# bayesian-object-tracking/dbot_ros

Measured on AMD Instinct MI355X. Metric: particle-likelihoods/sec @640x480, higher is better.
Workload: dtype f64; 1 GPU; C1: 2000 particles/GPU x loglikes(update=true), 640x480 synthetic depth frame, mesh m1 (5120 triangles), parents=permutation, 30-frame moving-object sequence, likelihood precision f64, window planes, inputs resident in HBM; particles_per_gpu=2000, triangles=5120

## Files before the change

dbot_ros_amd/csrc/rbsensor_kernels.hip:

```cpp
#pragma once
#include <hip/hip_runtime.h>
#include <math.h>
#include <stdint.h>

#include "rbs_device.h"
#include "rbs_math.h"

namespace rbs {

#ifndef RBS_TILE_PX
#define RBS_TILE_PX 11008
#endif
#ifndef RBS_COPY_UNROLL
#define RBS_COPY_UNROLL 8
#endif
#ifndef RBS_BIG_THRESH
#define RBS_BIG_THRESH 96
#endif

#ifndef RBS_BLOCK
#define RBS_BLOCK 256
#endif
constexpr int kBlock = RBS_BLOCK;
constexpr int kTilePx = RBS_TILE_PX;
// ... 1046 lines not shown
    RBS_EVAL_BATCH(qn);
#undef RBS_EVAL_BATCH
    RBS_TICK(3);
    if (draw && threadIdx.x == 0) ticket = atomicAdd(&P.ctr_this[1], 1);
    const double total = block_reduce_sum(ll, m.red);
    RBS_TICK(4);
    return total;
}

__device__ inline bool raster_writes(const DevParams& P, int particle, const int4& q, int row, int col)
{
    if (!(row >= q.y && row < q.w && col >= q.x && col < q.z)) return false;
    if (P.groups == nullptr) return true;
    const Groups* G = P.groups + particle;
    const int ng = G->n;
    for (int g = 0; g < ng; ++g) {
        const int4 r = G->rect[g];
        if (row >= r.y && row < r.w && col >= r.x && col < r.z) return true;
    }
    return false;
}

template <int VEC>
__device__ inline void copy_band(const DevParams& P, int particle, int band, Rect r)
{
    const int row0 = band * P.band_rows;
    const int row1 = min(P.rows, row0 + P.band_rows);
    if (row0 >= row1) return;
    const int parent = P.parents[particle];
    if ((unsigned)parent >= (unsigned)P.slots) return;
    const float* __restrict__ src = parent_plane(P, parent) + (size_t)row0 * P.cols;
    float* __restrict__ dst = P.occ_dst + (size_t)particle * P.plane_stride + (size_t)row0 * P.cols;
    const float alpha = P.alpha, beta = P.beta, bg_new = P.bg_new;

    if (VEC == 4) {
        const int W4 = P.cols >> 2;
        const int n4 = (row1 - row0) * W4;
        const floatx4* __restrict__ s4 = reinterpret_cast<const floatx4*>(src);
        floatx4* __restrict__ d4 = reinterpret_cast<floatx4*>(dst);
        const int qstep = kBlock / W4, rstep = kBlock - qstep * W4;
        int row = row0 + (int)threadIdx.x / W4;
        int c4 = (int)threadIdx.x - ((int)threadIdx.x / W4) * W4;
        for (int base = threadIdx.x; base < n4; base += kBlock * kCopyUnroll) {
            floatx4 v[kCopyUnroll];
            bool ok[kCopyUnroll];
#pragma unroll
            for (int k = 0; k < kCopyUnroll; ++k) {
                const int idx = base + k * kBlock;
                const int col = c4 << 2;
                ok[k] = idx < n4 && !raster_writes(P, particle, make_int4(r.x0, r.y0, r.x1, r.y1), row, col);
                if (ok[k]) v[k] = __builtin_nontemporal_load(&s4[idx]);
                c4 += rstep; row += qstep;
                if (c4 >= W4) { c4 -= W4; ++row; }
            }
#pragma unroll
            for (int k = 0; k < kCopyUnroll; ++k) {
                if (!ok[k]) continue;
                floatx4 w;
                w.x = occ_step(alpha, beta, v[k].x, bg_new);
                w.y = occ_step(alpha, beta, v[k].y, bg_new);
                w.z = occ_step(alpha, beta, v[k].z, bg_new);
                w.w = occ_step(alpha, beta, v[k].w, bg_new);
                __builtin_nontemporal_store(w, &d4[base + k * kBlock]);
            }
        }
    } else {
        const int W = P.cols;
        const int n1 = (row1 - row0) * W;
        for (int idx = threadIdx.x; idx < n1; idx += kBlock) {
            const int lr = idx / W;
            const int row = row0 + lr, col = idx - lr * W;
            if (raster_writes(P, particle, make_int4(r.x0, r.y0, r.x1, r.y1), row, col)) continue;
            dst[idx] = occ_step(alpha, beta, src[idx], bg_new);
        }
    }
}

constexpr int kPrepPerBlock = 8;

__device__ inline void compose_pose(const double* __restrict__ d, const double* __restrict__ d0, double* __restrict__ out)
{
    double Rd[9], R0[9];
    rbd::rotvec_to_matrix(d + 3, Rd);
    rbd::rotvec_to_matrix(d0 + 3, R0);
    rbd::matmul3(Rd, R0, out);
#pragma unroll
    for (int k = 0; k < 3; ++k) out[9 + k] = d[k] + d0[k];
}

template <bool DELTAS = false>
__device__ inline void prep_particles(const DevParams& P, int block, int* __restrict__ rects, int update)
{
    __shared__ int cnts[kPrepPerBlock + 1];
    const int w = threadIdx.x >> 6, lane = threadIdx.x & 63;
    const int i = block * kPrepPerBlock + w;
    const bool live = i < P.n;
    const int parent_early = live ? P.indices[i] : -1;
    Rect r = {0, 0, 0, 0};
    int cnt = 0;
    __shared__ int4 gr_s[kPrepPerBlock][kMaxBodies];
    __shared__ unsigned gm_s[kPrepPerBlock][kMaxBodies];
    __shared__ Groups G_s[kPrepPerBlock];
    __shared__ int ys_s[kPrepPerBlock][2 * kMaxGroups + 4];
    int4* const gr = gr_s[w];
    unsigned* const gm = gm_s[w];
    Groups& G = G_s[w];
    if (lane == 0) G.n = 0;
    const int cap_px = min(P.tile_w * P.tile_h, P.tile_px);
    if (DELTAS && live) {
        const int B = P.n_bodies;
        double* dstp = const_cast<double*>(P.poses) + (size_t)i * 12 * B;
        for (int b = lane; b < B; b += 64) {
            double d[6], d0[6], out[12];
#pragma unroll
            for (int k = 0; k < 6; ++k) { d[k] = P.deltas_src[((size_t)i * B + b) * 6 + k]; d0[k] = P.deltas_src[((size_t)P.n * B + b) * 6 + k]; }
            compose_pose(d, d0, out);
#pragma unroll
            for (int k = 0; k < 12; ++k) dstp[12 * b + k] = out[k];
        }
        __threadfence_block();
    } else if (P.poses_src && live) {
        const int m = 12 * P.n_bodies;
        double* dstp = const_cast<double*>(P.poses) + (size_t)i * m;
        const double* srcp = P.poses_src + (size_t)i * m;
        for (int k = lane; k < m; k += 64) dstp[k] = srcp[k];
        __threadfence_block();
    }
    if (live && P.groups == nullptr) {
        r = particle_rect(P, P.poses + (size_t)i * 12 * P.n_bodies);
        const TileGrid tg = tile_grid(r.x1 - r.x0, r.y1 - r.y0, P.tile_w, cap_px);
        cnt = r.x1 > r.x0 ? tg.nx * tg.ny : 1;
    } else if (live) {
        int ng = 0;
        for (int b = 0; b < P.n_bodies; ++b) {
            const Rect br = bodies_rect(P, P.poses + (size_t)i * 12 * P.n_bodies, b, b + 1);
            if (br.x1 > br.x0) {
                if (lane == 0) { gr[ng] = make_int4(br.x0, br.y0, br.x1, br.y1); gm[ng] = 1u << b; }
                ++ng;
            }
        }
        __builtin_amdgcn_wave_barrier();
        for (bool changed = true; changed;) {
            changed = false;
            for (int a = 0; a < ng && !changed; ++a)
                for (int c = a + 1; c < ng && !changed; ++c) {
                    const int4 A = gr[a], C = gr[c];
                    if (A.x < C.z && C.x < A.z && A.y < C.w && C.y < A.w) {
                        const int4 last = gr[ng - 1];
                        const unsigned ma = gm[a], mc = gm[c], ml = gm[ng - 1];
                        __builtin_amdgcn_wave_barrier();
                        if (lane == 0) {
                            gr[a] = make_int4(min(A.x, C.x), min(A.y, C.y), max(A.z, C.z), max(A.w, C.w));
                            gm[a] = ma | mc;
                            if (c != ng - 1) { gr[c] = last; gm[c] = ml; }
                        }
                        __builtin_amdgcn_wave_barrier();
                        --ng;
                        changed = true;
                    }
                }
        }
        if (ng > kMaxGroups) {
            int4 U = gr[0];
            unsigned mu = gm[0];
            for (int c = 1; c < ng; ++c) {
                const int4 C = gr[c];
                U = make_int4(min(U.x, C.x), min(U.y, C.y), max(U.z, C.z), max(U.w, C.w));
                mu |= gm[c];
            }
            __builtin_amdgcn_wave_barrier();
            if (lane == 0) { gr[0] = U; gm[0] = mu; }
            __builtin_amdgcn_wave_barrier();
            ng = 1;
        }
        if (lane == 0) G.n = ng;
        if (ng > 0) { const int4 g0 = gr[0]; r = Rect{g0.x, g0.y, g0.z, g0.w}; }
        for (int g = 0; g < ng; ++g) {
            const int4 R = gr[g];
            const TileGrid tg = tile_grid(R.z - R.x, R.w - R.y, P.tile_w, cap_px);
            if (lane == 0) { G.rect[g] = R; G.mask[g] = gm[g]; G.first[g] = cnt; }
            cnt += tg.nx * tg.ny;
            r.x0 = min(r.x0, R.x); r.y0 = min(r.y0, R.y);
            r.x1 = max(r.x1, R.z); r.y1 = max(r.y1, R.w);
        }
        if (ng == 0) cnt = 1;
    }
    if (lane == 0) cnts[w] = cnt;
    __syncthreads();
    if (threadIdx.x == 0) {
        int total = 0;
        for (int k = 0; k < kPrepPerBlock; ++k) { const int c = cnts[k]; cnts[k] = total; total += c; }
        cnts[kPrepPerBlock] = total ? atomicAdd(&P.ctr_this[0], total) : 0;
    }
    __syncthreads();
    if (!live || lane != 0) return;
    reinterpret_cast<int4*>(rects)[i] = make_int4(r.x0, r.y0, r.x1, r.y1);
    if (P.groups) {
        Groups* out = P.groups + i;
        out->n = G.n;
        for (int g = 0; g < G.n; ++g) { out->rect[g] = G.rect[g]; out->first[g] = G.first[g]; out->mask[g] = G.mask[g]; }
    }
    P.done[i] = 0;
    const int parent = parent_early;
    P.parents[i] = parent;
    const int first = cnts[kPrepPerBlock] + cnts[w];
    P.item_range[i] = make_int2(first, cnt);
    for (int k = 0; k < cnt; ++k) P.item_particle[first + k] = i;
    if (update && P.windowed) {
        const int4 rw = r.x1 > r.x0 ? make_int4(r.x0, r.y0, r.x1, r.y1) : make_int4(P.cols, P.rows, 0, 0);
        int4 pw = make_int4(P.cols, P.rows, 0, 0);
        if ((unsigned)parent < (unsigned)P.slots) pw = parent_window(P, parent);
        int4 u = make_int4(min(pw.x, rw.x), min(pw.y, rw.y), max(pw.z, rw.z), max(pw.w, rw.w));
        if (P.rebase_box) {
            const int4 bw = *P.rebase_box;
            u = make_int4(min(u.x, bw.x), min(u.y, bw.y), max(u.z, bw.z), max(u.w, bw.w));
        }
        int4 seed = rw;
        if (P.slab_px) {
            const long area = u.z > u.x && u.w > u.y ? (long)(u.z - u.x) * (long)(u.w - u.y) : 0;
            if (area > (long)P.err[1]) atomicMax(P.err + 1, (int)min(area, 0x7fffffffL));
            if (area > (long)P.slab_px) {
                P.parents[i] = -1;
                u = make_int4(P.cols, P.rows, 0, 0);
                seed = u;
                atomicExch(P.err, 1);
            }
            P.reg_dst[i] = u;
        }
        P.win_used[i] = u;
        P.win_dst[i] = seed;
        if (P.strips && P.groups) {
            Strips* S = P.strips + i;
            int* ys = ys_s[w];
            int ny = 0, ns = 0, total = 0;
            const int ng_ = G.n;
            if (u.z > u.x && u.w > u.y) {
                ys[ny++] = u.y;
                for (int g = 0; g < ng_; ++g) {
                    const int4 R = G.rect[g];
                    for (int e = 0; e < 2; ++e) {
                        const int y = min(max(e ? R.w : R.y, u.y), u.w);
                        int k = ny;
                        while (k > 0 && ys[k - 1] > y) --k;
                        if (k > 0 && ys[k - 1] == y) continue;
                        for (int m = ny; m > k; --m) ys[m] = ys[m - 1];
                        ys[k] = y; ++ny;
                    }
                }
                if (ys[ny - 1] != u.w) ys[ny++] = u.w;
                for (int bnd = 0; bnd + 1 < ny; ++bnd) {
                    const int ya = ys[bnd], yb = ys[bnd + 1];
                    int cur = u.x;
                    for (;;) {
                        int best = -1, bx = u.z;
                        for (int g = 0; g < ng_; ++g) {
                            const int4 R = G.rect[g];
                            if (R.z > R.x && R.y <= ya && R.w >= yb && R.z > cur && max(R.x, u.x) < bx) { best = g; bx = max(R.x, u.x); }
                        }
                        const int x1 = best < 0 ? u.z : bx;
                        if (x1 > cur) {
                            S->first[ns] = total;
                            S->box[ns] = make_ushort4((unsigned short)(cur >> 2), (unsigned short)(x1 >> 2), (unsigned short)ya, (unsigned short)yb);
                            total += ((x1 - cur) >> 2) * (yb - ya);
                            ++ns;
                        }
                        if (best < 0) break;
                        cur = max(cur, min(G.rect[best].z, u.z));
                        if (cur >= u.z) break;
                    }
                }
            }
            S->first[ns] = total;
            S->n = ns;
        }
        if (P.area_sum && (i & 7) == 0 && u.z > u.x && u.w > u.y)
            atomicAdd(P.area_sum, (unsigned long long)(u.z - u.x) * (unsigned long long)(u.w - u.y));
    }
}


__global__ __launch_bounds__(64 * kPrepPerBlock) void rbs_prep_kernel(const DevParams P, int* __restrict__ rects, int update)
{
    prep_particles(P, (int)blockIdx.x, rects, update);
}
__global__ __launch_bounds__(64 * kPrepPerBlock) void rbs_prep_deltas_kernel(const DevParams P, int* __restrict__ rects, int update)
{
    prep_particles<true>(P, (int)blockIdx.x, rects, update);
}

__global__ __launch_bounds__(64 * kPrepPerBlock) void rbs_frame_prep_kernel(const DevParams P, int* __restrict__ rects, int update,
                                      const float* __restrict__ frame_src, double* __restrict__ aux,
                                      float* __restrict__ pbg, float* __restrict__ keep, int aux_blocks)
{
    const int prep_blocks = (int)gridDim.x - aux_blocks;
    if ((int)blockIdx.x < prep_blocks) {
        prep_particles(P, (int)blockIdx.x, rects, update);
    } else {
        const int i = ((int)blockIdx.x - prep_blocks) * (int)blockDim.x + (int)threadIdx.x;
        if (i < P.npx) frame_aux_pixel(i, frame_src, aux, pbg, P.npx, P.tw, P.ms, P.sf, P.lambda, keep);
    }
}

#ifndef RBS_FCOPY_UNROLL
#define RBS_FCOPY_UNROLL 2
#endif
__device__ __forceinline__ void fused_window_copy(const DevParams& P, int particle)
{
    constexpr int kU = RBS_FCOPY_UNROLL;
    const int parent = P.parents[particle];
    if ((unsigned)parent >= (unsigned)P.slots) return;
    const int4 u = P.win_used[particle];
    if (u.z <= u.x || u.w <= u.y) return;
    const int4 q = reinterpret_cast<const int4*>(P.rects)[particle];
    const bool has = q.z > q.x;
    const int w4 = (u.z - u.x) >> 2, ux4 = u.x >> 2, W4 = P.cols >> 2;
    const int ty1 = has ? q.y : u.w, tby0 = has ? q.w : u.w;
    const int left4 = has ? (q.x - u.x) >> 2 : 0, right4 = has ? (u.z - q.z) >> 2 : 0, m = left4 + right4;
    const int rjump = has ? (q.z - u.x) >> 2 : 0;
    const int n_top = (ty1 - u.y) * w4, n_mid = (tby0 - ty1) * m, L = n_top + n_mid + (u.w - tby0) * w4;
    if (L == 0) return;
    const float rw4 = 1.0f / (float)w4, rm = 1.0f / (float)max(m, 1);
    const int4 pw = parent_window(P, parent);
    const floatx4* __restrict__ s4 = reinterpret_cast<const floatx4*>(parent_plane(P, parent));
    floatx4* __restrict__ d4 = reinterpret_cast<floatx4*>(P.occ_dst + (size_t)particle * P.plane_stride);
    const float alpha = P.alpha, beta = P.beta, bg_new = P.bg_new;
    int bx0 = P.cols, by0 = P.rows, bx1 = 0, by1 = 0;
    for (int base = 0; base < L; base += kBlock * kU) {
        floatx4 v[kU];
        int pk[kU];
#pragma unroll
        for (int k = 0; k < kU; ++k) {
            const int idx = base + k * kBlock + (int)threadIdx.x;
            const bool live = idx < L;
            const bool top = idx < n_top, mid = !top && idx < n_top + n_mid;
            const int j = top ? idx : mid ? idx - n_top : idx - n_top - n_mid, d = mid ? m : w4;
            int r = (int)((float)j * (mid ? rm : rw4));
            r += (r + 1) * d <= j ? 1 : 0;
            r -= r * d > j ? 1 : 0;
            const int kk = j - r * d;
            const int row = (top ? u.y : mid ? ty1 : tby0) + r, c4 = mid ? (kk < left4 ? kk : kk - left4 + rjump) : kk;
            const int col = (ux4 + c4) << 2;
            const bool stored = live && col >= pw.x && col < pw.z && row >= pw.y && row < pw.w;
            pk[k] = ((live ? (stored ? 2 : 1) : 0) << 28) | (row << 14) | (ux4 + c4);
            if (stored) v[k] = __builtin_nontemporal_load(&s4[row * W4 + (ux4 + c4)]);
        }
#pragma unroll
        for (int k = 0; k < kU; ++k) {
            const int st_ = pk[k] >> 28, row_ = (pk[k] >> 14) & 0x3fff, at_ = pk[k] & 0x3fff;
            if (!st_) continue;
            floatx4 w;
            if (st_ == 2) {
                w.x = occ_step(alpha, beta, v[k].x, bg_new);
                w.y = occ_step(alpha, beta, v[k].y, bg_new);
                w.z = occ_step(alpha, beta, v[k].z, bg_new);
                w.w = occ_step(alpha, beta, v[k].w, bg_new);
            } else {
                w.x = w.y = w.z = w.w = bg_new;
            }
            __builtin_nontemporal_store(w, &d4[row_ * W4 + at_]);
            if (w.x != bg_new || w.y != bg_new || w.z != bg_new || w.w != bg_new) {
                const int col = at_ << 2;
                bx0 = min(bx0, col); bx1 = max(bx1, col + 4);
                by0 = min(by0, row_); by1 = max(by1, row_ + 1);
            }
        }
    }
#pragma unroll
    for (int off = 32; off > 0; off >>= 1) {
        bx0 = min(bx0, __shfl_xor(bx0, off)); by0 = min(by0, __shfl_xor(by0, off));
        bx1 = max(bx1, __shfl_xor(bx1, off)); by1 = max(by1, __shfl_xor(by1, off));
    }
    if ((threadIdx.x & 63) == 0 && bx1 > bx0) {
        int* wd = reinterpret_cast<int*>(&P.win_dst[particle]);
        atomicMin(wd + 0, bx0); atomicMin(wd + 1, by0);
        atomicMax(wd + 2, bx1); atomicMax(wd + 3, by1);
    }
}

#ifndef RBS_RASTER_MINWAVES_F64
#define RBS_RASTER_MINWAVES_F64 3
#endif
#ifndef RBS_RASTER_MINWAVES
#define RBS_RASTER_MINWAVES 3
#endif
constexpr size_t smem_bytes(int tile_px, bool math_tables, bool many = false, bool exact = false);
template <bool UPDATE, int PREC, bool SLAB, bool MANY = false, bool STP = false, bool EXACT = false, bool ONE = false, bool FCOPY = false>
__device__ __forceinline__ void raster_kernel_body(const DevParams& P)
{
    static_assert(!FCOPY || (UPDATE && !SLAB && !MANY && !STP && !EXACT), "the fused copy serves windowed whole planes, scalar background");
    extern __shared__ __attribute__((aligned(16))) unsigned char smem[];
    Smem m = carve(smem, P.tile_px, PREC == 0);
    if (EXACT) {
        m.ageq = reinterpret_cast<int*>(smem + smem_bytes(P.tile_px, PREC == 0, MANY));
        m.agetab = reinterpret_cast<double*>(m.ageq + (kBlock / 64) * kEvalQueue);
        for (int i = threadIdx.x; i < 2 * min(kLdsAges, P.age_max + 1); i += kBlock) m.agetab[i] = P.ptab[i];
    }
    const int total = P.ctr_this[0];
    if (blockIdx.x == 0 && threadIdx.x == 0) { P.ctr_next[0] = 0; P.ctr_next[1] = 0; }
    if (PREC == 0) {
        constexpr int ne = rbsm::kErfcIntervals * rbsm::kErfcCoefs, nl = rbsm::kLogIntervals * 2;
        for (int i = threadIdx.x; i < ne; i += kBlock) m.mtab[i] = rbsm::kErfcTab[i];
        for (int i = threadIdx.x; i < nl; i += kBlock) m.mtab[ne + i] = rbsm::kLogTab[i];
    }
#ifdef RBS_PHASE_TIMING
    const unsigned long long c0_ = clock64(), w0_ = wall_clock64();
    if (threadIdx.x < 32) g_phase_lds[threadIdx.x] = 0;
#endif
    RBS_TICK_DECL;
    const int grid = (int)gridDim.x;
    const int static_end = grid;
    int item = (int)blockIdx.x;
    for (;;) {
        if (item >= total) break;
        RBS_TICK(7);
        const int particle = __builtin_amdgcn_readfirstlane(P.item_particle[item]);
        const int4 q = reinterpret_cast<const int4*>(P.rects)[particle];
        const Rect r = {q.x, q.y, q.z, q.w};
        const int2 range = P.item_range[particle];
        const int first = range.x;
        double part = 0.0;
        const bool draw = item + grid >= static_end;
        int ticket = -1;
#ifdef RBS_PHASE_TIMING
        if (threadIdx.x == 0 && q.x + range.y == -12345) P.out[0] = 0.0;
        RBS_TICK(15);
#endif
        if (ONE || P.groups == nullptr) {
            if (r.x1 > r.x0) part = raster_eval_tile<UPDATE, PREC, SLAB, MANY, 0, STP, EXACT, ONE>(P, particle, r, item - first, m, 0xffffffffu, draw, ticket);
        } else {
            const Groups* G = P.groups + particle;
            const int k = item - first, ng = __builtin_amdgcn_readfirstlane(G->n);
            int g = 0;
            for (int c = 1; c < ng; ++c) g += (k >= __builtin_amdgcn_readfirstlane(G->first[c])) ? 1 : 0;
            if (ng > 0) {
                const int4 gq = G->rect[g];
                const Rect gr = {__builtin_amdgcn_readfirstlane(gq.x), __builtin_amdgcn_readfirstlane(gq.y),
                                 __builtin_amdgcn_readfirstlane(gq.z), __builtin_amdgcn_readfirstlane(gq.w)};
                part = raster_eval_tile<UPDATE, PREC, SLAB, MANY, 0, STP, EXACT>(P, particle, gr, k - __builtin_amdgcn_readfirstlane(G->first[g]), m,
                                                      (unsigned)__builtin_amdgcn_readfirstlane((int)G->mask[g]), draw, ticket);
            }
        }
        if (threadIdx.x == 0) {
            const int cnt = range.y;
            if (cnt == 1) {
                P.out[particle] = part;
            } else {
                unsigned long long* pp = reinterpret_cast<unsigned long long*>(P.partial);
                const unsigned long long old = atomicExch(pp + item, (unsigned long long)__double_as_longlong(part));
                const int bump = old == 0xfff8deadbeef0000ull ? 2 : 1;
                if (atomicAdd(&P.done[particle], bump) == cnt - 1) {
                    double sum = 0.0;
                    for (int k = 0; k < cnt; ++k) sum += __longlong_as_double((long long)atomicOr(pp + first + k, 0ull));
                    P.out[particle] = sum;
                }
            }
        }
        if (FCOPY && item == first) fused_window_copy(P, particle);
        if (draw) {
            if (threadIdx.x == 0) {
                if (ticket < 0) ticket = atomicAdd(&P.ctr_this[1], 1);
                *m.item = static_end + ticket;
            }
            __syncthreads();
            item = __builtin_amdgcn_readfirstlane(*m.item);
        } else {
            item += grid;
            __syncthreads();
        }
#ifdef RBS_PHASE_TIMING
        tick_ = clock64();
#endif
    }
#ifdef RBS_PHASE_TIMING
    if (threadIdx.x == 0) {
        for (int k = 0; k < 32; ++k)
            if (k != 5 && k != 6) atomicAdd(&P.phase[k], g_phase_lds[k]);
        atomicAdd(&P.phase[5], clock64() - c0_);
        atomicAdd(&P.phase[6], wall_clock64() - w0_);
    }
#endif
}

template <bool UPDATE, bool SLAB>
__global__ __launch_bounds__(kBlock, RBS_RASTER_MINWAVES) __attribute__((amdgpu_num_vgpr(RBS_RASTER_VGPRS)))
void rbs_raster_kernel_f32(const DevParams P)
{
    raster_kernel_body<UPDATE, 1, SLAB>(P);
}
#ifndef RBS_RASTER_VGPRS_F64
#define RBS_RASTER_VGPRS_F64 80
#endif
#define RBS_F64_BUDGET __attribute__((amdgpu_num_vgpr(RBS_RASTER_VGPRS_F64)))
template <bool UPDATE, bool SLAB>
__global__ __launch_bounds__(kBlock, RBS_RASTER_MINWAVES_F64) RBS_F64_BUDGET void rbs_raster_kernel_f64(const DevParams P)
{
    raster_kernel_body<UPDATE, 0, SLAB>(P);
}
template <bool UPDATE, bool SLAB>
__global__ __launch_bounds__(kBlock, RBS_RASTER_MINWAVES_F64) RBS_F64_BUDGET void rbs_raster_kernel_one_f64(const DevParams P)
{
    raster_kernel_body<UPDATE, 0, SLAB, false, false, false, true>(P);
}
__global__ __launch_bounds__(kBlock, RBS_RASTER_MINWAVES_F64) RBS_F64_BUDGET void rbs_raster_kernel_wcopy_one_f64(const DevParams P)
{
    raster_kernel_body<true, 0, false, false, false, false, true, true>(P);
}
__global__ __launch_bounds__(kBlock, RBS_RASTER_MINWAVES) __attribute__((amdgpu_num_vgpr(RBS_RASTER_VGPRS)))
void rbs_raster_kernel_wcopy_f32(const DevParams P)
{
    raster_kernel_body<true, 1, false, false, false, false, false, true>(P);
}
template <bool UPDATE, bool SLAB, bool MANY>
__global__ __launch_bounds__(kBlock, RBS_RASTER_MINWAVES_F64) RBS_F64_BUDGET void rbs_raster_kernel_stp_f64(const DevParams P)
{
    raster_kernel_body<UPDATE, 0, SLAB, MANY, true>(P);
}
template <bool UPDATE, bool SLAB, bool MANY>
__global__ __launch_bounds__(kBlock, RBS_RASTER_MINWAVES) __attribute__((amdgpu_num_vgpr(RBS_RASTER_VGPRS)))
void rbs_raster_kernel_stp_f32(const DevParams P)
{
    raster_kernel_body<UPDATE, 1, SLAB, MANY, true>(P);
}
template <bool UPDATE, bool SLAB, bool MANY, bool STP>
__global__ __launch_bounds__(kBlock, RBS_RASTER_MINWAVES_F64) RBS_F64_BUDGET void rbs_raster_kernel_exact_f64(const DevParams P)
{
    raster_kernel_body<UPDATE, 0, SLAB, MANY, STP, true>(P);
}
template <bool UPDATE, bool SLAB, bool STP>
__global__ __launch_bounds__(kBlock, RBS_RASTER_MINWAVES_F64) RBS_F64_BUDGET void rbs_raster_kernel_exact_one_f64(const DevParams P)
{
    raster_kernel_body<UPDATE, 0, SLAB, false, STP, true, true>(P);
}
template <bool UPDATE, bool SLAB>
__global__ __launch_bounds__(kBlock, RBS_RASTER_MINWAVES) __attribute__((amdgpu_num_vgpr(RBS_RASTER_VGPRS)))
void rbs_raster_kernel_many_f32(const DevParams P)
{
    raster_kernel_body<UPDATE, 1, SLAB, true>(P);
}
template <bool UPDATE, bool SLAB>
__global__ __launch_bounds__(kBlock, RBS_RASTER_MINWAVES_F64) RBS_F64_BUDGET void rbs_raster_kernel_many_f64(const DevParams P)
{
    raster_kernel_body<UPDATE, 0, SLAB, true>(P);
}

#ifndef RBS_DEPTH_TILE_PX
#define RBS_DEPTH_TILE_PX kTilePxF64
#endif
#ifndef RBS_DEPTH_MINWAVES
#define RBS_DEPTH_MINWAVES 3
#endif
#ifndef RBS_DEPTH_VGPRS
#define RBS_DEPTH_VGPRS 80
#endif
#ifndef RBS_EVAL_MINWAVES
#define RBS_EVAL_MINWAVES 4
#endif
constexpr int kDepthTilePx = RBS_DEPTH_TILE_PX;
static_assert(kDepthTilePx == kTilePxF64 || RBS_DEPTH_MINWAVES != 3, "the split launch shares the one-kernel launch's tile");
struct SmemDepth { unsigned* tile; int* big; int* nbig; int* item; int* tq; unsigned long long* cull; };
__device__ inline SmemDepth carve_depth(unsigned char* smem, int tile_px)
{
    SmemDepth m;
    m.tile = reinterpret_cast<unsigned*>(smem);
    m.big = reinterpret_cast<int*>(smem + sizeof(unsigned) * tile_px);
    m.nbig = m.big + kBigCap;
    m.item = m.nbig + 1;
    m.tq = m.nbig + 4;
    m.cull = reinterpret_cast<unsigned long long*>(m.tq + kTq * (kBlock / 64));
    return m;
}
constexpr size_t smem_bytes_depth(int tile_px, bool many)
{
    return sizeof(unsigned) * (size_t)tile_px + sizeof(int) * kBigCap + 16 + sizeof(int) * kTq * (kBlock / 64) + (many ? 16 * kCullSteps : 0);
}
static_assert(RBS_DEPTH_MINWAVES * ((smem_bytes_depth(kDepthTilePx, true) + 1279) / 1280 * 1280) <= 160 * 1024, "the geometry kernel's blocks per CU");

template <bool MANY>
__device__ __forceinline__ void depth_kernel_body(const DevParams& P)
{
    extern __shared__ __attribute__((aligned(16))) unsigned char smem[];
    const SmemDepth m = carve_depth(smem, P.tile_px);
    const int total = P.ctr_this[0];
    if (blockIdx.x == 0 && threadIdx.x == 0) { P.ctr_next[0] = 0; P.ctr_next[1] = 0; *P.ctrb_this = 0; *P.ctrb_next = 0; }
    const int grid = (int)gridDim.x;
    int item = (int)blockIdx.x;
    for (;;) {
        if (item >= total) break;
        const int particle = __builtin_amdgcn_readfirstlane(P.item_particle[item]);
        const int first = P.item_range[particle].x;
        Rect r;
        unsigned body_mask = 0xffffffffu;
        int tile_id = item - first;
        bool have;
        if (P.groups == nullptr) {
            const int4 q = reinterpret_cast<const int4*>(P.rects)[particle];
            r = Rect{q.x, q.y, q.z, q.w};
            have = r.x1 > r.x0;
        } else {
            const Groups* G = P.groups + particle;
            const int ng = __builtin_amdgcn_readfirstlane(G->n);
            int g = 0;
            for (int c = 1; c < ng; ++c) g += (tile_id >= __builtin_amdgcn_readfirstlane(G->first[c])) ? 1 : 0;
            have = ng > 0;
            r = Rect{0, 0, 0, 0};
            if (have) {
                const int4 gq = G->rect[g];
                r = Rect{__builtin_amdgcn_readfirstlane(gq.x), __builtin_amdgcn_readfirstlane(gq.y),
                         __builtin_amdgcn_readfirstlane(gq.z), __builtin_amdgcn_readfirstlane(gq.w)};
                tile_id -= __builtin_amdgcn_readfirstlane(G->first[g]);
                body_mask = (unsigned)__builtin_amdgcn_readfirstlane((int)G->mask[g]);
            }
        }
        const int parent = P.parents[particle];
        if (have && (unsigned)parent < (unsigned)P.slots && item < P.depth_items) {
            const TileGrid tg = tile_grid(r.x1 - r.x0, r.y1 - r.y0, P.tile_w, min(P.tile_w * P.tile_h, P.tile_px));
            const int ty = tile_id / tg.nx, tx = tile_id - ty * tg.nx;
            const int wx0 = r.x0 + tx * tg.tw, wy0 = r.y0 + ty * tg.th;
            const int wx1 = min(r.x1, wx0 + tg.tw), wy1 = min(r.y1, wy0 + tg.th);
            const int npx = (wx1 - wx0) * (wy1 - wy0);
            const bool whole = (wx0 == r.x0 && wy0 == r.y0 && wx1 == r.x1 && wy1 == r.y1);
            const double* pose = P.poses + (size_t)particle * 12 * P.n_bodies;
            raster_window<MANY>(P, pose, wx0, wy0, wx1, wy1, !whole || (body_mask & (body_mask - 1u)) != 0u, m.tile, m.big, m.nbig,
                                m.tq + (threadIdx.x >> 6) * kTq, body_mask, m.cull);
            unsigned* __restrict__ out = P.depth + (size_t)item * P.tile_px;
            if ((npx & 3) == 0) {
                const uint4* __restrict__ t4 = reinterpret_cast<const uint4*>(m.tile);
                uint4* __restrict__ o4 = reinterpret_cast<uint4*>(out);
                for (int k = threadIdx.x; k < (npx >> 2); k += kBlock) o4[k] = t4[k];
            } else {
                for (int k = threadIdx.x; k < npx; k += kBlock) out[k] = m.tile[k];
            }
        }
        if (threadIdx.x == 0) *m.item = grid + atomicAdd(&P.ctr_this[1], 1);
        __syncthreads();
        item = __builtin_amdgcn_readfirstlane(*m.item);
        __syncthreads();
    }
}
template <bool MANY>
__global__ __launch_bounds__(kBlock, RBS_DEPTH_MINWAVES) __attribute__((amdgpu_num_vgpr(RBS_DEPTH_VGPRS)))
void rbs_depth_kernel(const DevParams P)
{
    depth_kernel_body<MANY>(P);
}

template <bool UPDATE, bool SLAB, bool STP = false, bool EXACT = false>
__global__ __launch_bounds__(kBlock, RBS_EVAL_MINWAVES) void rbs_eval_kernel(const DevParams P)
{
    extern __shared__ __attribute__((aligned(16))) unsigned char smem[];
    Smem m = carve(smem, 0, true);
    if (EXACT) {
        m.ageq = reinterpret_cast<int*>(smem + smem_bytes(0, true, false));
        m.agetab = reinterpret_cast<double*>(m.ageq + (kBlock / 64) * kEvalQueue);
        for (int i = threadIdx.x; i < 2 * min(kLdsAges, P.age_max + 1); i += kBlock) m.agetab[i] = P.ptab[i];
    }
    const int total = P.ctr_this[0];
    {
        constexpr int ne = rbsm::kErfcIntervals * rbsm::kErfcCoefs, nl = rbsm::kLogIntervals * 2;
        for (int i = threadIdx.x; i < ne; i += kBlock) m.mtab[i] = rbsm::kErfcTab[i];
        for (int i = threadIdx.x; i < nl; i += kBlock) m.mtab[ne + i] = rbsm::kLogTab[i];
    }
    __syncthreads();
    const int grid = (int)gridDim.x;
    int item = (int)blockIdx.x;
    for (;;) {
        if (item >= total) break;
        const int particle = __builtin_amdgcn_readfirstlane(P.item_particle[item]);
// ... 550 lines not shown
```

Before: 10.82 million particle-likelihoods/s.

## Restructure fused window copy into column-fixed row loops per region

```diff
diff --git a/dbot_ros_amd/csrc/rbsensor_kernels.hip b/dbot_ros_amd/csrc/rbsensor_kernels.hip
--- a/dbot_ros_amd/csrc/rbsensor_kernels.hip
+++ b/dbot_ros_amd/csrc/rbsensor_kernels.hip
@@ -1372,7 +1372,7 @@
 }
 
 #ifndef RBS_FCOPY_UNROLL
-#define RBS_FCOPY_UNROLL 2
+#define RBS_FCOPY_UNROLL 4
 #endif
 __device__ __forceinline__ void fused_window_copy(const DevParams& P, int particle)
 {
@@ -1387,52 +1387,58 @@
     const int ty1 = has ? q.y : u.w, tby0 = has ? q.w : u.w;
     const int left4 = has ? (q.x - u.x) >> 2 : 0, right4 = has ? (u.z - q.z) >> 2 : 0, m = left4 + right4;
     const int rjump = has ? (q.z - u.x) >> 2 : 0;
-    const int n_top = (ty1 - u.y) * w4, n_mid = (tby0 - ty1) * m, L = n_top + n_mid + (u.w - tby0) * w4;
-    if (L == 0) return;
-    const float rw4 = 1.0f / (float)w4, rm = 1.0f / (float)max(m, 1);
+    const int n_above = ty1 - u.y, n_full = n_above + (u.w - tby0), n_side = tby0 - ty1;
+    if (n_full * w4 + n_side * m == 0) return;
     const int4 pw = parent_window(P, parent);
     const floatx4* __restrict__ s4 = reinterpret_cast<const floatx4*>(parent_plane(P, parent));
     floatx4* __restrict__ d4 = reinterpret_cast<floatx4*>(P.occ_dst + (size_t)particle * P.plane_stride);
     const float alpha = P.alpha, beta = P.beta, bg_new = P.bg_new;
+    const int tid = (int)threadIdx.x;
     int bx0 = P.cols, by0 = P.rows, bx1 = 0, by1 = 0;
-    for (int base = 0; base < L; base += kBlock * kU) {
-        floatx4 v[kU];
-        int pk[kU];
-#pragma unroll
-        for (int k = 0; k < kU; ++k) {
-            const int idx = base + k * kBlock + (int)threadIdx.x;
-            const bool live = idx < L;
-            const bool top = idx < n_top, mid = !top && idx < n_top + n_mid;
-            const int j = top ? idx : mid ? idx - n_top : idx - n_top - n_mid, d = mid ? m : w4;
-            int r = (int)((float)j * (mid ? rm : rw4));
-            r += (r + 1) * d <= j ? 1 : 0;
-            r -= r * d > j ? 1 : 0;
-            const int kk = j - r * d;
-            const int row = (top ? u.y : mid ? ty1 : tby0) + r, c4 = mid ? (kk < left4 ? kk : kk - left4 + rjump) : kk;
-            const int col = (ux4 + c4) << 2;
-            const bool stored = live && col >= pw.x && col < pw.z && row >= pw.y && row < pw.w;
-            pk[k] = ((live ? (stored ? 2 : 1) : 0) << 28) | (row << 14) | (ux4 + c4);
-            if (stored) v[k] = __builtin_nontemporal_load(&s4[row * W4 + (ux4 + c4)]);
-        }
-#pragma unroll
-        for (int k = 0; k < kU; ++k) {
-            const int st_ = pk[k] >> 28, row_ = (pk[k] >> 14) & 0x3fff, at_ = pk[k] & 0x3fff;
-            if (!st_) continue;
-            floatx4 w;
-            if (st_ == 2) {
-                w.x = occ_step(alpha, beta, v[k].x, bg_new);
-                w.y = occ_step(alpha, beta, v[k].y, bg_new);
-                w.z = occ_step(alpha, beta, v[k].z, bg_new);
-                w.w = occ_step(alpha, beta, v[k].w, bg_new);
-            } else {
-                w.x = w.y = w.z = w.w = bg_new;
-            }
-            __builtin_nontemporal_store(w, &d4[row_ * W4 + at_]);
-            if (w.x != bg_new || w.y != bg_new || w.z != bg_new || w.w != bg_new) {
-                const int col = at_ << 2;
-                bx0 = min(bx0, col); bx1 = max(bx1, col + 4);
-                by0 = min(by0, row_); by1 = max(by1, row_ + 1);
-            }
+#pragma nounroll
+    for (int side = 0; side < 2; ++side) {
+        const int width = side ? m : w4, nrows = side ? n_side : n_full;
+        if (width <= 0 || nrows <= 0) continue;
+        const int row0 = side ? ty1 : u.y, tsplit = side ? nrows : n_above, rskip = tby0 - ty1;
+        const int csplit = side ? left4 : width, cjump = rjump - left4;
+        const int R = width >= kBlock ? 1 : kBlock / width;
+        const int lr = width >= kBlock ? 0 : tid / width, lc = tid - lr * width;
+        for (int c0 = 0; c0 < width; c0 += kBlock) {
+            const int c = c0 + lc;
+            const bool on = lr < R && c < width;
+            const int at = ux4 + c + (c >= csplit ? cjump : 0), col = at << 2;
+            const bool in_pw = on && col >= pw.x && col < pw.z;
+            bool hit = false;
+            auto cell = [&](auto* plane, int row) { return plane + (unsigned)(row * W4 + at); };
+            for (int t0 = 0; t0 < nrows; t0 += R * kU) {
+                floatx4 v[kU];
+#pragma unroll
+                for (int k = 0; k < kU; ++k) {
+                    const int t = t0 + k * R + lr, row = row0 + t + (t >= tsplit ? rskip : 0);
+                    if (in_pw && t < nrows && row >= pw.y && row < pw.w) v[k] = __builtin_nontemporal_load(cell(s4, row));
+                }
+                __builtin_amdgcn_s_waitcnt(0x0f70);
+#pragma unroll
+                for (int k = 0; k < kU; ++k) {
+                    const int t = t0 + k * R + lr, row = row0 + t + (t >= tsplit ? rskip : 0);
+                    if (!on || t >= nrows) continue;
+                    floatx4 w;
+                    if (in_pw && row >= pw.y && row < pw.w) {
+                        w.x = occ_step(alpha, beta, v[k].x, bg_new);
+                        w.y = occ_step(alpha, beta, v[k].y, bg_new);
+                        w.z = occ_step(alpha, beta, v[k].z, bg_new);
+                        w.w = occ_step(alpha, beta, v[k].w, bg_new);
+                    } else {
+                        w.x = w.y = w.z = w.w = bg_new;
+                    }
+                    __builtin_nontemporal_store(w, cell(d4, row));
+                    if (w.x != bg_new || w.y != bg_new || w.z != bg_new || w.w != bg_new) {
+                        hit = true;
+                        by0 = min(by0, row); by1 = max(by1, row + 1);
+                    }
+                }
+            }
+            if (hit) { bx0 = min(bx0, col); bx1 = max(bx1, col + 4); }
         }
     }
 #pragma unroll
```

Measured after the change: 10.95 million particle-likelihoods/s, median of 6. 1.2% higher.
